# rust-bio/rust-bio

Measured on AMD Instinct MI355X. Metric: GCUPS (SW) + FM-index queries/sec, higher is better.
Workload: dtype int16; 1 GPU; 1000000 x 150 bp synthetic read pairs per GPU, Aligner::local affine-gap (-5,-1,+1,-1), score+coords+traceback ops (BASELINE configs[1]); pairs_per_gpu=1000000, read_len=150, parallelism=shard1

## Files before the change

rust-bio_amd/csrc/bg_common.h:

```cpp
#ifndef BG_COMMON_H
#define BG_COMMON_H
#include <functional>
#include <hip/hip_runtime.h>

#include <cstdint>
#include <cstdlib>
#include <cstdio>
#include <cstring>
#include <string>
#include <vector>

#include "biogpu.h"

extern thread_local std::string bg_tls_error;

#define BG_HIP(call)                                                                     \
    do {                                                                                 \
        hipError_t e__ = (call);                                                         \
        if (e__ != hipSuccess) {                                                         \
            bg_tls_error = std::string(#call) + ": " + hipGetErrorString(e__);           \
            return e__ == hipErrorOutOfMemory ? BG_ERR_OOM : BG_ERR_HIP;                 \
        }                                                                                \
    } while (0)

struct bg_band_scratch;
void bg_band_scratch_free(bg_band_scratch*);
struct bg_seed_scratch;
void bg_seed_scratch_free(bg_seed_scratch*);
struct bg_host_pipe;
void bg_host_pipe_free(bg_host_pipe*);
struct bg_fm_pipe;
void bg_fm_pipe_free(bg_fm_pipe*);
struct bg_myers_scratch;
void bg_myers_scratch_free(bg_myers_scratch*);

struct bg_ctx {
    int device = 0;
    hipStream_t stream = nullptr;
    void* tb = nullptr;
    size_t tb_bytes = 0;
    void* aux = nullptr;
    size_t aux_bytes = 0;
    void* bnd = nullptr;
    size_t bnd_bytes = 0;
    void* io[6] = {};
    size_t io_cap[6] = {};
    void* h_ops = nullptr;
    size_t h_ops_cap = 0;
    void* unpk[2] = {};
    size_t unpk_cap[2] = {};
    void* table = nullptr;
    size_t table_bytes = 0;
    void* sw_table = nullptr;
    size_t sw_table_bytes = 0;
    uint64_t table_hash = 0;
    int table_alpha = 0;
    int32_t* table_matrix = nullptr;
    bg_band_scratch* band = nullptr;
    bg_host_pipe* pipe = nullptr;
    bg_seed_scratch* seed = nullptr;
    bg_fm_pipe* fm_pipe = nullptr;
    bg_myers_scratch* myers = nullptr;
    int64_t myers_chunk_jobs = 0;
    int64_t myers_lds_bytes = 0;
    uint64_t fm_wide_from = 0xFFFFFFFFull;
    uint32_t fm_wide_sb_shift = 17;
    bool fm_host_bytes = false;
    int64_t host_chunk_pairs = 0;
    int64_t chunk_pairs = 0;
    int64_t seed_chunk_reads = 0;
    bool force_wide = false;
    bool no_pk16 = false;
    bool no_local_fast = false;
    bool no_pk16_frame = false;
    bool no_couples = false;
    int band_chain_global = -1;
    bool fq_no_fused = false;
    int sam_lanes = 0;
    int fq_emit_mode = 0;
    int64_t sa_chunk_symbols = 0;
    bool band_chain_rows = true;
    bool band_join_global = false;
    int band_fill_v1 = 0;
    bool band_interior_off = false;
    bool band_packed_off = false;
    int64_t band_packed_thresh = 0;
    int64_t band_budget_gb = 0;
    bool band_on_host = false;
    hipEvent_t scratch_done = nullptr;
    hipStream_t scratch_stream = nullptr;
    bool scratch_used = false;
    bool timing = false;
    hipEvent_t ev[2] = {nullptr, nullptr};
    bg_timing_t last = {};
    uint32_t fill_mask = 0;
    bool fill_framed = false;
};

int bg_reserve(void** p, size_t* cur, size_t need);
int bg_scan_u32(const uint32_t* d_len, uint64_t n, uint64_t* d_off, uint64_t* d_sums, hipStream_t st);
int bg_align_batch_dev_hint(bg_ctx* ctx, const bg_scoring_t* sc, int mode, uint64_t n_pairs, const uint8_t* d_x,
                            const uint64_t* d_x_off, const uint8_t* d_y, const uint64_t* d_y_off, uint32_t max_xlen,
                            uint32_t max_ylen, bg_alignment_t* d_out, uint8_t* d_ops, uint64_t ops_stride, void* stream,
                            int len_hint);

size_t bg_compact_ops_scratch(uint64_t n);
int bg_range_to_host(const uint8_t* d_src, uint8_t* h_dst, const uint64_t* d_slot , hipStream_t st);
int bg_compact_ops_dev(bg_alignment_t* d_rec, uint64_t n, const uint8_t* d_ops, uint8_t* d_compact, bool global_offsets, uint64_t* d_cell,
                       uint64_t* d_batch_total, void* d_scratch, bool long_ops, hipStream_t st);

struct bg_scratch_guard {
    bg_ctx* ctx;
    hipStream_t st;
    bg_scratch_guard(bg_ctx* c, hipStream_t s) : ctx(c), st(s) {
        if (ctx->scratch_used && ctx->scratch_stream != st) hipStreamWaitEvent(st, ctx->scratch_done, 0);
    }
    ~bg_scratch_guard() {
        if (hipEventRecord(ctx->scratch_done, st) == hipSuccess) {
            ctx->scratch_stream = st;
            ctx->scratch_used = true;
        }
    }
};
inline hipError_t bg_copy_pieces(void* dst, const void* src, size_t bytes, hipMemcpyKind kind, hipStream_t st) {
    static const size_t piece = [] {
        const char* e = getenv("BG_COPY_PIECE");
        const long long v = e ? atoll(e) : 0;
// ... 30 lines not shown
```

rust-bio_amd/csrc/core.hip:

```cpp
#include <sched.h>

#include <algorithm>
#include <condition_variable>
#include <deque>
#include <mutex>
#include <thread>

#include <cstdlib>

#include "bg_common.h"

thread_local std::string bg_tls_error;

int bg_reserve(void** p, size_t* cur, size_t need) {
    if (need <= *cur) return BG_OK;
    if (*p) {
        hipFree(*p);
        *p = nullptr;
        *cur = 0;
    }
    need = (need + 255) & ~(size_t)255;
    BG_HIP(hipMalloc(p, need));
    *cur = need;
    return BG_OK;
// ... 198 lines not shown
    }
    if (!strcmp(key, "myers_lds_bytes")) {
        if (value != 0 && (value < 4096 || value > 65536)) return BG_ERR_INVALID_ARG;
        ctx->myers_lds_bytes = value;
        return BG_OK;
    }
    if (!strcmp(key, "sa_chunk_symbols")) {
        if (value < 0) return BG_ERR_INVALID_ARG;
        ctx->sa_chunk_symbols = value;
        return BG_OK;
    }
    if (!strcmp(key, "band_chain_rows")) {
        ctx->band_chain_rows = value != 0;
        return BG_OK;
    }
    if (!strcmp(key, "band_chain_global")) {
        ctx->band_chain_global = (int)value;
        return BG_OK;
    }
    if (!strcmp(key, "band_fill_v1")) {
        ctx->band_fill_v1 = value > 0 ? 1 : value < 0 ? -1 : 0;
        return BG_OK;
    }
    if (!strcmp(key, "band_interior_off")) {
        ctx->band_interior_off = value != 0;
        return BG_OK;
    }
    if (!strcmp(key, "band_packed_off")) {
        ctx->band_packed_off = value != 0;
        return BG_OK;
    }
    if (!strcmp(key, "band_packed_thresh")) {
        if (value < 0 || value > 0xffff) return BG_ERR_INVALID_ARG;
        ctx->band_packed_thresh = value;
        return BG_OK;
    }
    if (!strcmp(key, "band_budget_gb")) {
        if (value < 0 || value > 256) return BG_ERR_INVALID_ARG;
        ctx->band_budget_gb = value;
        return BG_OK;
    }
    if (!strcmp(key, "band_on_host")) {
        ctx->band_on_host = value != 0;
        return BG_OK;
    }
    if (!strcmp(key, "fm_host_bytes")) {
        ctx->fm_host_bytes = value != 0;
        return BG_OK;
    }
    if (!strcmp(key, "host_chunk_pairs")) {
        ctx->host_chunk_pairs = value;
        return BG_OK;
    }
    if (!strcmp(key, "no_couples")) {
        ctx->no_couples = value != 0;
        return BG_OK;
    }
    if (!strcmp(key, "no_local_fast")) {
        ctx->no_local_fast = value != 0;
        return BG_OK;
    }
    if (!strcmp(key, "no_pk16_frame")) {
        ctx->no_pk16_frame = value != 0;
        return BG_OK;
    }
    if (!strcmp(key, "no_pk16")) {
        ctx->no_pk16 = value != 0;
        return BG_OK;
    }
    if (!strcmp(key, "force_wide")) {
        ctx->force_wide = value != 0;
        return BG_OK;
    }
    return BG_ERR_INVALID_ARG;
}

extern "C" int bg_enable_timing(bg_ctx* ctx, int on) {
    if (!ctx) return BG_ERR_INVALID_ARG;
    ctx->timing = on != 0;
    ctx->last = {};
    return BG_OK;
}

extern "C" int bg_last_fill_kernels(bg_ctx* ctx, uint32_t* mask) {
    if (!ctx || !mask) return BG_ERR_INVALID_ARG;
    *mask = ctx->fill_mask;
    return BG_OK;
}

extern "C" int bg_last_fill_framed(bg_ctx* ctx, int* framed) {
    if (!ctx || !framed) return BG_ERR_INVALID_ARG;
    *framed = ctx->fill_framed ? 1 : 0;
    return BG_OK;
}

extern "C" int bg_get_timing(bg_ctx* ctx, bg_timing_t* out) {
    if (!ctx || !out) return BG_ERR_INVALID_ARG;
    *out = ctx->last;
    ctx->last = {};
    return BG_OK;
}

namespace {
__global__ __launch_bounds__(256) void ops_counts_kernel(const bg_alignment_t* __restrict__ rec, uint64_t n, uint32_t* __restrict__ cnt) {
    const uint64_t p = (uint64_t)blockIdx.x * blockDim.x + threadIdx.x;
    if (p < n) cnt[p] = rec[p].status == BG_OK ? rec[p].n_ops : 0u;
// ... 62 lines not shown
```

rust-bio_amd/csrc/sw_api.hip:

```cpp
#include <algorithm>
#include <chrono>
#include <map>
#include <type_traits>

#include <atomic>
#include <condition_variable>
#include <mutex>
#include <thread>

#include "sw_kernels.h"

namespace bgsw {
void launch_traceback(const SwArgs& a, int nw, hipStream_t st);

static sw_fill_fn sw_fill_get(SwFill f, bool narrow, int lp, int r, int which = 0) {
    static sw_fill_fn (*const get[])(bool, int, int, int) = {
#define BG_X(F) sw_fill_get_##F,
        BG_SW_FILLS(BG_X)
#undef BG_X
    };
    return get[f](narrow, lp, r, which);
}
static int instantiated_r(SwFill f, bool narrow, int lp, int r0, uint32_t m = 0) {
    for (int r = r0; r <= 12; r++)
        if ((!m || m % r == 0) && sw_fill_get(f, narrow, lp, r)) return r;
    return 0;
}

struct Config {
    int lp, r;
};
static Config pick_config(uint32_t m_cap) {
    if (m_cap <= 192) return {16, std::max(2, 2 * (int)((m_cap + 31) / 32))};
    if (m_cap <= 384) return {32, std::max(8, 2 * (int)((m_cap + 63) / 64))};
    return {64, 8};
}

static int64_t score_magnitude(const SwScoring& c, const int32_t* matrix) {
    int64_t mag = std::max<int64_t>(std::abs((int64_t)c.go), std::abs((int64_t)c.ge));
    for (int32_t v : {c.xp, c.xs, c.yp, c.ys})
        if (v != BG_MIN_SCORE) mag = std::max<int64_t>(mag, std::abs((int64_t)v));
    if (matrix) {
        for (size_t t = 0; t < 65536; t++) mag = std::max<int64_t>(mag, std::abs((int64_t)matrix[t]));
    } else {
        mag = std::max<int64_t>(mag, std::max(std::abs((int64_t)c.match), std::abs((int64_t)c.mismatch)));
    }
    return mag;
}

struct FillPlan {
    int lp = 0, r = 0;
    sw_fill_fn fill = nullptr, fill_rest = nullptr, fill_second = nullptr;
    uint32_t tb_fmt = TBF_K1;
    uint32_t fill_bit = 0;
    bool k1p = false, framed = false;
};
static FillPlan plan_fill(const bg_ctx& ctx, const SwScoring& c, int sm, int64_t mag, uint32_t max_xlen, uint32_t max_ylen) {
    const Config cfg = pick_config(max_xlen);
    const bool local = c.xp == 0 && c.xs == 0 && c.yp == 0 && c.ys == 0;
    const bool lf = local && c.go < 0 && c.mismatch < 0 && c.match >= 0 && !ctx.no_local_fast;
    FillPlan p;
    p.lp = cfg.lp;
    if (!ctx.no_pk16 && sm == SCORE_PARAMS && cfg.lp <= 32 && max_xlen >= 1 && mag * ((int64_t)std::max(max_xlen, max_ylen) + 2) <= 2040) {
        const int32_t M = BG_MIN_SCORE;
        SwFill f = lf      ? FILL_K1P_LF
                   : local ? FILL_K1P_LOCAL
// ... 157 lines not shown
        const uint32_t u = threadIdx.x >= (unsigned)o ? s[threadIdx.x - o] : 0;
        __syncthreads();
        s[threadIdx.x] += u;
        __syncthreads();
    }
    cnt[blockIdx.x * 1024u + threadIdx.x] = base + s[threadIdx.x] - v;
}
__global__ __launch_bounds__(256) void sw_key_scatter_kernel(const uint64_t* __restrict__ x_off, const uint64_t* __restrict__ y_off, uint64_t pair0,
                                                             uint32_t n, uint32_t* __restrict__ cursor, uint32_t* __restrict__ perm,
                                                             const uint32_t* __restrict__ st) {
    if (st && st[0] == st[2] && st[1] == st[3]) return;
    const uint32_t p = blockIdx.x * blockDim.x + threadIdx.x;
    const bool valid = p < n;
    uint32_t base;
    const uint32_t rank = wave_key_add(cursor, valid ? len_key(x_off, y_off, pair0 + p) : 0u, valid, base);
    if (valid) perm[base + rank] = p;
}
__global__ void sw_decide_kernel(const uint32_t* __restrict__ st, uint32_t n, int forced, uint32_t* __restrict__ n_eff) {
    const bool uniform = forced < 0 && st[0] == st[2] && st[1] == st[3];
    n_eff[0] = uniform ? n : 0u;
    n_eff[1] = uniform ? 0u : n;
}
}

using namespace bgsw;

int bg_compact_matrix(const int32_t* matrix, std::vector<uint8_t>& code_map, std::vector<int32_t>& table) {
    return compact_matrix(matrix, code_map, table);
}

static int check_scoring(const bg_scoring_t* sc) {
    if (sc->gap_open > 0 || sc->gap_extend > 0 || sc->xclip_prefix > 0 || sc->xclip_suffix > 0 ||
        sc->yclip_prefix > 0 || sc->yclip_suffix > 0)
        return BG_ERR_POSITIVE_PENALTY;
    return BG_OK;
}

static void reset_fill_report(bg_ctx* ctx) {
    if (!ctx) return;
    ctx->fill_mask = 0;
    ctx->fill_framed = false;
}

static int align_batch_dev_impl(bg_ctx* ctx, const bg_scoring_t* sc, int mode, uint64_t n_pairs,
                                const uint8_t* d_x, const uint64_t* d_x_off, const uint8_t* d_y,
                                const uint64_t* d_y_off, uint32_t max_xlen, uint32_t max_ylen,
                                bg_alignment_t* d_out, uint8_t* d_ops, uint64_t ops_stride,
                                void* stream, int len_hint, const uint8_t* packed_codes = nullptr) {
    if (!ctx || !sc || mode < BG_MODE_CUSTOM || mode > BG_MODE_LOCAL) return BG_ERR_INVALID_ARG;
    int rc = check_scoring(sc);
    if (rc) return rc;
    if (n_pairs == 0) return BG_OK;
    if (!d_x_off || !d_y_off || !d_out) return BG_ERR_INVALID_ARG;
    if (d_ops && ops_stride < (uint64_t)max_xlen + max_ylen + 4) return BG_ERR_OPS_CAP;
    if (max_xlen > (1u << 24) || max_ylen > (1u << 24)) return BG_ERR_TOO_LARGE;
    hipStream_t st = (hipStream_t)stream;
    BG_HIP(hipSetDevice(ctx->device));
    bg_scratch_guard guard(ctx, st);

    SwArgs a = {};
    a.x = d_x;
    a.x_off = d_x_off;
    a.y = d_y;
    a.y_off = d_y_off;
    a.sc = {sc->gap_open,     sc->gap_extend,   sc->xclip_prefix, sc->xclip_suffix,
            sc->yclip_prefix, sc->yclip_suffix, sc->match_score,  sc->mismatch_score};
    if (mode == BG_MODE_GLOBAL) a.sc.xp = a.sc.xs = a.sc.yp = a.sc.ys = BG_MIN_SCORE;
    if (mode == BG_MODE_SEMIGLOBAL) {
        a.sc.xp = a.sc.xs = BG_MIN_SCORE;
        a.sc.yp = a.sc.ys = 0;
    }
    if (mode == BG_MODE_LOCAL) a.sc.xp = a.sc.xs = a.sc.yp = a.sc.ys = 0;
    a.mode = mode;
    a.filter_clips = (mode == BG_MODE_SEMIGLOBAL || mode == BG_MODE_LOCAL);
    a.out = d_out;
    a.ops = d_ops;
    a.ops_stride = ops_stride;

    int sm = SCORE_PARAMS;
    if (sc->matrix) {
        uint64_t h = 0xcbf29ce484222325ull;
        {
            const uint64_t* w = (const uint64_t*)sc->matrix;
            uint64_t h2 = 0x9e3779b97f4a7c15ull;
            for (size_t t = 0; t < 32768; t += 2) {
                h = (h ^ w[t]) * 0x100000001b3ull;
                h2 = (h2 + w[t + 1]) * 0xff51afd7ed558ccdull;
                h2 ^= h2 >> 32;
            }
            h ^= h2;
            if (h == 0) h = 1;
        }
        if (ctx->table_hash != h || !ctx->table_matrix || memcmp(ctx->table_matrix, sc->matrix, 65536 * sizeof(int32_t)) != 0) {
            std::vector<uint8_t> code_map;
            std::vector<int32_t> table;
            const int A = compact_matrix(sc->matrix, code_map, table);
            const size_t bytes = 256 + table.size() * 4;
            ctx->table_hash = 0;
            if (!ctx->table_matrix && !(ctx->table_matrix = (int32_t*)malloc(65536 * sizeof(int32_t)))) return BG_ERR_OOM;
            if ((rc = bg_reserve(&ctx->sw_table, &ctx->sw_table_bytes, bytes))) return rc;
            BG_HIP(hipMemcpyAsync((uint8_t*)ctx->sw_table + 256, table.data(), table.size() * 4,
                                  hipMemcpyHostToDevice, st));
            BG_HIP(hipMemcpyAsync(ctx->sw_table, code_map.data(), 256, hipMemcpyHostToDevice, st));
            BG_HIP(hipStreamSynchronize(st));
            memcpy(ctx->table_matrix, sc->matrix, 65536 * sizeof(int32_t));
            ctx->table_hash = h;
            ctx->table_alpha = A;
// ... 58 lines not shown
    uint32_t *d_keycnt = nullptr, *d_keysum = nullptr, *d_perm = nullptr, *d_lenst = nullptr;
    if (plan.k1p && !ctx->no_couples) {
        const size_t need = (size_t)kLenKeys * 4 + 1024 * 4 + 64 + chunk * 4;
        if ((rc = bg_reserve(&ctx->bnd, &ctx->bnd_bytes, need))) return rc;
        a.bnd = (int4*)ctx->bnd;
        d_keycnt = (uint32_t*)ctx->bnd;
        d_keysum = d_keycnt + kLenKeys;
        d_lenst = d_keysum + 1024;
        d_perm = d_lenst + 16;
    }

    for (uint64_t p0 = 0; p0 < n_pairs; p0 += chunk) {
        a.pair0 = p0;
        a.n_pairs = (uint32_t)std::min<uint64_t>(chunk, n_pairs - p0);
        const uint32_t njobs = (a.n_pairs + pw - 1) / pw;
        a.perm = nullptr;
        a.len_stats = nullptr;
        a.n_eff = nullptr;
        if (d_perm && a.n_pairs >= 64 && len_hint != 1) {
            const uint32_t* d_st = nullptr;
            if (len_hint < 0) {
                BG_HIP(hipMemsetAsync(d_lenst, 0xff, 8, st));
                BG_HIP(hipMemsetAsync(d_lenst + 2, 0, 8, st));
                sw_len_stats_kernel<<<dim3(std::min<uint32_t>((a.n_pairs + 255) / 256, 256)), dim3(256), 0, st>>>(d_x_off, d_y_off, p0, a.n_pairs, d_lenst);
                d_st = d_lenst;
            }
            BG_HIP(hipMemsetAsync(d_keycnt, 0, (size_t)kLenKeys * 4, st));
            sw_key_hist_kernel<<<dim3((a.n_pairs + 255) / 256), dim3(256), 0, st>>>(d_x_off, d_y_off, p0, a.n_pairs, d_keycnt, d_st);
            sw_key_block_sums_kernel<<<dim3(1024), dim3(256), 0, st>>>(d_keycnt, d_keysum, d_st);
            sw_key_scan_kernel<<<dim3(1024), dim3(1024), 0, st>>>(d_keycnt, d_keysum, d_st);
            sw_key_scatter_kernel<<<dim3((a.n_pairs + 255) / 256), dim3(256), 0, st>>>(d_x_off, d_y_off, p0, a.n_pairs, d_keycnt, d_perm, d_st);
            BG_HIP(hipGetLastError());
            sw_decide_kernel<<<dim3(1), dim3(1), 0, st>>>(d_lenst, a.n_pairs, len_hint < 0 ? -1 : 0, d_lenst + 4);
            a.perm = d_perm;
            a.len_stats = d_st;
            a.n_eff = d_lenst + 4;
        }
        if (ctx->timing) BG_HIP(hipEventRecord(ctx->ev[0], st));
        const uint32_t nwaves = plan.k1p ? (njobs + 1) / 2 : njobs;
        plan.fill<<<dim3((nwaves + 3) / 4), dim3(256), 0, st>>>(a);
        BG_HIP(hipGetLastError());
        if (ctx->timing) BG_HIP(hipEventRecord(ctx->ev[1], st));
        if (plan.fill_rest) plan.fill_rest<<<dim3((nwaves + 3) / 4), dim3(256), 0, st>>>(a);
        if (plan.fill_second && len_hint != 1) plan.fill_second<<<dim3((nwaves + 3) / 4), dim3(256), 0, st>>>(a);
        BG_HIP(hipGetLastError());
        if (ctx->timing) {
            BG_HIP(hipEventSynchronize(ctx->ev[1]));
            float ms = 0;
            BG_HIP(hipEventElapsedTime(&ms, ctx->ev[0], ctx->ev[1]));
            ctx->last.fill_ms += ms;
            ctx->last.fill_launches += 1;
            BG_HIP(hipEventRecord(ctx->ev[0], st));
        }
        launch_traceback(a, nw, st);
        BG_HIP(hipGetLastError());
        if (ctx->timing) {
            BG_HIP(hipEventRecord(ctx->ev[1], st));
            BG_HIP(hipEventSynchronize(ctx->ev[1]));
            float ms = 0;
            BG_HIP(hipEventElapsedTime(&ms, ctx->ev[0], ctx->ev[1]));
            ctx->last.traceback_ms += ms;
            ctx->last.traceback_launches += 1;
        }
    }
    return BG_OK;
}

int bg_align_batch_dev_hint(bg_ctx* ctx, const bg_scoring_t* sc, int mode, uint64_t n_pairs, const uint8_t* d_x,
                            const uint64_t* d_x_off, const uint8_t* d_y, const uint64_t* d_y_off, uint32_t max_xlen,
                            uint32_t max_ylen, bg_alignment_t* d_out, uint8_t* d_ops, uint64_t ops_stride, void* stream,
                            int len_hint) {
    return align_batch_dev_impl(ctx, sc, mode, n_pairs, d_x, d_x_off, d_y, d_y_off, max_xlen, max_ylen, d_out, d_ops, ops_stride,
                                stream, len_hint);
}

extern "C" int bg_align_batch_dev(bg_ctx* ctx, const bg_scoring_t* sc, int mode, uint64_t n_pairs,
                                  const uint8_t* d_x, const uint64_t* d_x_off, const uint8_t* d_y,
                                  const uint64_t* d_y_off, uint32_t max_xlen, uint32_t max_ylen,
                                  bg_alignment_t* d_out, uint8_t* d_ops, uint64_t ops_stride,
                                  void* stream) {
    reset_fill_report(ctx);
    return align_batch_dev_impl(ctx, sc, mode, n_pairs, d_x, d_x_off, d_y, d_y_off, max_xlen, max_ylen, d_out, d_ops, ops_stride, stream, -1);
}

extern "C" int bg_align_batch_packed_dev(bg_ctx* ctx, const bg_scoring_t* sc, int mode, uint64_t n_pairs, const uint32_t* d_x,
                                         const uint64_t* d_x_off, const uint32_t* d_y, const uint64_t* d_y_off,
                                         const uint8_t codes[4], uint32_t max_xlen, uint32_t max_ylen, bg_alignment_t* d_out,
                                         uint8_t* d_ops, uint64_t ops_stride, void* stream) {
    if (!codes || (n_pairs && (!d_x || !d_y))) return BG_ERR_INVALID_ARG;
    for (int a = 0; a < 4; a++)
        for (int b = a + 1; b < 4; b++)
            if (codes[a] == codes[b]) return BG_ERR_INVALID_ARG;
    reset_fill_report(ctx);
    return align_batch_dev_impl(ctx, sc, mode, n_pairs, (const uint8_t*)d_x, d_x_off, (const uint8_t*)d_y, d_y_off, max_xlen, max_ylen,
                                d_out, d_ops, ops_stride, stream, -1, codes);
}

struct bg_host_pipe {
    static constexpr int NSET = 3;
    struct Set {
        uint8_t *h_in = nullptr, *h_out = nullptr;
        uint8_t *d_in = nullptr, *d_out = nullptr;
        uint8_t *d_cmp = nullptr, *d_scan = nullptr;
        size_t in_cap = 0, out_cap = 0, cmp_cap = 0, scan_cap = 0;
        hipEvent_t in_done = nullptr, k_done = nullptr, out_done = nullptr;
    } set[NSET];
    uint64_t* d_cell = nullptr;
// ... 374 lines not shown
```

rust-bio_amd/csrc/sw_kernels.h:

```cpp
#ifndef BG_SW_KERNELS_H
#define BG_SW_KERNELS_H
#include <type_traits>

#include "bg_common.h"

namespace bgsw {

constexpr int32_t NEG = BG_MIN_SCORE;

enum : uint32_t {
    TB_START = 0, TB_INS = 1, TB_DEL = 2, TB_SUBST = 3, TB_MATCH = 4,
    TB_XCLIP_PREFIX = 5, TB_XCLIP_SUFFIX = 6, TB_YCLIP_PREFIX = 7, TB_YCLIP_SUFFIX = 8
};
enum : uint32_t { C_XS = 7, C_MATCH = 6, C_SUBST = 5, C_INS = 3, C_DEL = 2, C_XP = 1, C_YP = 0 };
constexpr int32_t kNarrowFloor = -(1 << 26);
constexpr int32_t kNarrowKeyFloor = (int32_t)0x80000000;

enum { SCORE_PARAMS = 0, SCORE_LDS = 1, SCORE_GLOBAL = 2 };
constexpr int kMaxLdsAlphabet = 64;

struct SwScoring {
    int32_t go, ge, xp, xs, yp, ys;
    int32_t match, mismatch;
};
// ... 112 lines not shown
    }
    if (sc.xp > c.S) {
        c.S = sc.xp;
        c.sbits = TB_XCLIP_PREFIX;
    }
    return c;
}
__device__ __forceinline__ void col0_fold(const SwScoring& sc, uint32_t m, int32_t& fold, uint32_t& lx0) {
    fold = NEG;
    lx0 = 0;
    if (m >= 2) {
        const Col0 c = col0_cell(sc, 1, m, NEG);
        if (c.S + sc.xs > fold) {
            fold = c.S + sc.xs;
            lx0 = m - 1;
        }
    }
}
__device__ __forceinline__ int32_t col0_S(const SwScoring& sc, uint32_t i, uint32_t m, int32_t fold0) {
    if (i == 0) return 0;
    return col0_cell(sc, i, m, fold0).S;
}

struct Row0 {
    int32_t S, D;
    uint32_t sbits, dbits;
};
__device__ __forceinline__ Row0 row0_cell(const SwScoring& sc, uint32_t j) {
    Row0 c;
    if (j == 1) {
        c.D = sc.go;
        c.dbits = TB_START;
    } else {
        const int32_t d_score = sc.go + sc.ge * ((int32_t)j - 1);
        const int32_t c_score = sc.yp + sc.go;
        if (d_score > c_score) {
            c.D = d_score;
            c.dbits = TB_DEL;
        } else {
            c.D = c_score;
            c.dbits = TB_YCLIP_PREFIX;
        }
    }
    if (c.D > sc.yp) {
        c.S = c.D;
        c.sbits = TB_DEL;
    } else {
        c.S = sc.yp;
        c.sbits = TB_YCLIP_PREFIX;
    }
    return c;
}

__device__ __forceinline__ uint32_t s_nibble_of_code(uint32_t code) {
    switch (code) {
        case C_MATCH: return TB_MATCH;
        case C_SUBST: return TB_SUBST;
        case C_INS: return TB_INS;
        case C_DEL: return TB_DEL;
        case C_XP: return TB_XCLIP_PREFIX;
        case C_YP: return TB_YCLIP_PREFIX;
        default: return TB_XCLIP_SUFFIX;
    }
}

typedef void (*sw_fill_fn)(const SwArgs);

#define BG_K1_SHAPES(X) X(16, 2) X(16, 4) X(16, 6) X(16, 8) X(16, 10) X(16, 12) X(32, 8) X(32, 10) X(32, 12) X(64, 8)
#define BG_K1_TABLE_SHAPES(X) X(16, 6) X(16, 12) X(32, 12) X(64, 8)
#define BG_K1_TABLE_LDS_NARROW_SHAPES(X) BG_K1_TABLE_SHAPES(X) X(16, 8) X(16, 10)
#define BG_K1P_SHAPES(X) X(16, 2) X(16, 4) X(16, 5) X(16, 6) X(16, 8) X(16, 10) X(16, 12) X(32, 8) X(32, 10) X(32, 12)
#define BG_K1P_LOCAL_SHAPES(X)                                                                                    \
    X(16, 2) X(16, 3) X(16, 4) X(16, 5) X(16, 6) X(16, 7) X(16, 8) X(16, 9) X(16, 10) X(16, 11) X(16, 12) \
    X(32, 7) X(32, 8) X(32, 9) X(32, 10) X(32, 11) X(32, 12)

#define BG_SW_FILLS(X) \
    X(K1) X(K1_LOCAL) X(K1_LF) X(K1_LDS) X(K1_LDS_LOCAL) X(K1_GLOBAL) X(K1P_CUSTOM) X(K1P_GLOBAL) X(K1P_SEMIGLOBAL) X(K1P_LOCAL) X(K1P_LF) X(K1P_LF_FRAMED)
enum SwFill {
#define BG_X(F) FILL_##F,
    BG_SW_FILLS(BG_X)
#undef BG_X
};
#define BG_X(F) sw_fill_fn sw_fill_get_##F(bool narrow, int lp, int r, int which);
BG_SW_FILLS(BG_X)
#undef BG_X

}
#endif
```

rust-bio_amd/csrc/sw_traceback.hip:

```cpp
#include "sw_kernels.h"

namespace bgsw {

constexpr uint32_t kSegStride = 20;

template <int NW, bool PERM>
__global__ __launch_bounds__(256) __attribute__((amdgpu_waves_per_eu(5, 5))) void sw_traceback_kernel(const SwArgs a) {
    const uint32_t slot = blockIdx.x * blockDim.x + threadIdx.x;
    if (slot >= (a.n_eff ? a.n_eff[PERM ? 1 : 0] : a.n_pairs)) return;
    const uint32_t pair = PERM ? a.perm[slot] : slot;
    const SwScoring sc = a.sc;
    const SwGeom geo = a.g;
    const uint32_t R = geo.r, LP = geo.lp, PW = 64 / geo.lp;

    const uint64_t xo = a.x_off[a.pair0 + pair], yo = a.y_off[a.pair0 + pair];
    const uint32_t m = (uint32_t)(a.x_off[a.pair0 + pair + 1] - xo);
    const uint32_t n = (uint32_t)(a.y_off[a.pair0 + pair + 1] - yo);
    if (len_over(geo, m, n)) {
        bg_alignment_t bad = {};
        bad.xlen = m;
        bad.ylen = n;
        bad.ops_off = (a.pair0 + pair + 1) * a.ops_stride;
        bad.mode = (uint8_t)a.mode;
        bad.status = (int8_t)BG_ERR_INVALID_ARG;
        a.out[a.pair0 + pair] = bad;
        return;
    }

    const int32_t* aux = a.aux + (size_t)slot * geo.aux_stride;
    const int32_t* gLy = aux + geo.off_Ly();
    const int32_t* gLx = aux + geo.off_Lx();
    const uint8_t* bits = (const uint8_t*)(aux + geo.off_bits());
    const uint32_t sbits_m0 = (uint32_t)aux[0];
    const int32_t score = aux[1];
    const uint32_t lxn = (uint32_t)aux[2];

    const uint32_t job = slot / PW, grp = slot % PW;
    const uint32_t* tbj = (const uint32_t*)a.tb + (size_t)job * tb_job_words(geo.nstrips, geo.nsteps, NW);
    __shared__ __align__(16) uint32_t s_seg[256 * kSegStride];
    uint32_t* seg = s_seg + threadIdx.x * kSegStride;
    uint64_t seg_tag = ~0ull;
    auto cell = [&](uint32_t i, uint32_t j) -> uint32_t {
        const uint32_t i1 = i - 1, lrow = __umulhi(i1, geo.r_inv), rr = i1 - lrow * R;
        const uint32_t st = lrow >> geo.lp_shift, llc = lrow & (LP - 1);
        const uint64_t g = (uint64_t)st * geo.nsteps + (j - 1 + llc);
        constexpr uint32_t tsteps = 16 / NW;
        const uint64_t base = (g / tsteps) * 1024ull + (grp * LP + llc) * 16u;
        if (base != seg_tag) {
#pragma unroll
            for (int q = 0; q < 4; q++) *(uint4*)&seg[4 * q] = *(const uint4*)&tbj[base + 4 * q];
            seg_tag = base;
        }
        const uint32_t w = seg[(uint32_t)(g % tsteps) * NW + rr / 6];
        const uint32_t c = rr % 6;
        if (geo.tb_fmt == TBF_K1) return (w >> (5 * c)) & 31u;
        if (geo.tb_fmt == TBF_K1_LF) {
            const uint32_t u = (w >> (5 * c)) & 31u;
            return ((u >> 1) & 7u) | ((~u & 1u) << 3) | (~u & 16u);
        }
        const uint32_t v = (w >> (5 * (c % 3) + 16 * (c / 3))) & 31u;
        const uint32_t mv = (v >> 1) & 7u;
        return ((geo.tb_fmt == TBF_K1P_LF && mv == 0) ? (uint32_t)C_XP : mv) | ((v & 1u) << 3) | (v & 16u);
    };
    auto s_fill = [&](uint32_t i, uint32_t j) -> uint32_t {
        if (j == 0) {
            if (i == 0) return TB_START;
            if (i == m) return sbits_m0;
            return col0_cell(sc, i, m, NEG).sbits;
        }
        if (i == 0) return row0_cell(sc, j).sbits;
        return s_nibble_of_code(cell(i, j) & 7u);
    };
    auto s_nib = [&](uint32_t i, uint32_t j) -> uint32_t {
        if (j == n) return (uint32_t)bits[i] & 15u;
        return s_fill(i, j);
    };
    auto i_nib = [&](uint32_t i, uint32_t j) -> uint32_t {
        if (j == n) return (uint32_t)bits[i] >> 4;
        if (i == 0) return TB_START;
        if (j == 0) return col0_cell(sc, i, m, NEG).ibits;
        return (cell(i, j) & 8u) ? TB_INS : s_fill(i - 1, j);
    };
    auto d_nib = [&](uint32_t i, uint32_t j) -> uint32_t {
        if (j == 0) return TB_START;
        if (i == 0) return row0_cell(sc, j).dbits;
        return (cell(i, j) & 16u) ? TB_DEL : s_fill(i, j - 1);
    };

    uint8_t* ops_end = a.ops ? a.ops + (a.pair0 + pair + 1) * a.ops_stride : nullptr;
    uint32_t n_ops = 0;
    uint32_t clip_len[4] = {0, 0, 0, 0};
    uint32_t n_clips = 0;
    int status = BG_OK;
    const bool dword_ok = ops_end && (((uintptr_t)ops_end & 3) == 0);
    uint32_t acc = 0;
    auto push = [&](uint32_t op) {
        ++n_ops;
        if (!ops_end) return;
        if (dword_ok) {
            acc = (acc << 8) | op;
            if ((n_ops & 3) == 0) *(uint32_t*)(ops_end - n_ops) = acc;
        } else {
            ops_end[-(int64_t)n_ops] = (uint8_t)op;
        }
    };
    auto push_clip = [&](uint32_t op, uint32_t len) {
        if (a.filter_clips) return;
        if (n_clips < 4) clip_len[n_clips] = len;
        else status = BG_ERR_TRACEBACK;
        n_clips++;
        push(op);
    };

    uint32_t i = m, j = n;
    uint32_t xstart = 0, ystart = 0, xend = m, yend = n;
    uint32_t layer = s_nib(m, n);
    const uint32_t guard = 2 * (m + n) + 16;
    uint32_t c_here = 0;
    bool have_c = false;
    for (uint32_t steps = 0; layer != TB_START; steps++) {
        if (steps > guard || (ops_end && n_ops + 1 > a.ops_stride)) {
            status = BG_ERR_TRACEBACK;
            break;
        }
        if (layer >= TB_INS && layer <= TB_MATCH && i >= 1 && i <= m && j >= 1 && j < n) {
            const bool is_ins = layer == TB_INS, is_del = layer == TB_DEL;
            const uint32_t ti = i - (is_del ? 0u : 1u), tj = j - (is_ins ? 0u : 1u);
            if (ti >= 1 && tj >= 1) {
                if (!have_c && (is_ins || is_del)) c_here = cell(i, j);
                const bool ext = (is_ins && (c_here & 8u)) || (is_del && (c_here & 16u));
                push(is_ins ? (uint32_t)BG_OP_INS : is_del ? (uint32_t)BG_OP_DEL : layer == TB_MATCH ? (uint32_t)BG_OP_MATCH : (uint32_t)BG_OP_SUBST);
                c_here = cell(ti, tj);
                have_c = true;
                if (!ext) layer = s_nibble_of_code(c_here & 7u);
                i = ti;
                j = tj;
                continue;
            }
        }
        have_c = false;
        uint32_t next;
        switch (layer) {
            case TB_INS:
                push(BG_OP_INS);
                next = i_nib(i, j);
                i -= 1;
                break;
            case TB_DEL:
                push(BG_OP_DEL);
                next = d_nib(i, j);
                j -= 1;
                break;
            case TB_MATCH:
            case TB_SUBST:
                push(layer == TB_MATCH ? BG_OP_MATCH : BG_OP_SUBST);
                next = (i && j) ? s_nib(i - 1, j - 1) : TB_START;
                i -= 1;
                j -= 1;
                break;
            case TB_XCLIP_PREFIX:
                push_clip(BG_OP_XCLIP, i);
                xstart = i;
                i = 0;
                next = s_nib(0, j);
                break;
            case TB_XCLIP_SUFFIX: {
                if ((geo.tb_fmt == TBF_K1P_LF || geo.tb_fmt == TBF_K1_LF) && j != n) {
                    status = BG_ERR_TRACEBACK;
                    layer = TB_START;
                    continue;
                }
                const uint32_t lx = (j == n) ? lxn
                                    : geo.tb_fmt == TBF_K1 ? (uint32_t)gLx[j]
                                    : geo.lp == 16 ? (uint32_t)((const uint8_t*)gLx)[j] : (uint32_t)((const uint16_t*)gLx)[j];
                push_clip(BG_OP_XCLIP, lx);
                i -= lx;
                xend = i;
                next = i <= m ? s_nib(i, j) : TB_START;
                break;
            }
            case TB_YCLIP_PREFIX:
                push_clip(BG_OP_YCLIP, j);
                ystart = j;
                j = 0;
                next = s_nib(i, 0);
                break;
            default: {
                const uint32_t ly = (uint32_t)gLy[i];
                push_clip(BG_OP_YCLIP, ly);
                j -= ly;
                yend = j;
                next = j <= n ? s_nib(i, j) : TB_START;
                break;
            }
        }
        if (i > m || j > n) {
            status = BG_ERR_TRACEBACK;
            break;
        }
        layer = next;
    }

    if (dword_ok) {
        const uint32_t k = n_ops & 3, done = n_ops - k;
        for (uint32_t t = 0; t < k; t++) ops_end[-(int64_t)(done + t + 1)] = (uint8_t)(acc >> (8 * (k - 1 - t)));
    }
    bg_alignment_t rec;
    rec.score = score;
    rec.xstart = xstart;
    rec.xend = xend;
    rec.ystart = ystart;
    rec.yend = yend;
    rec.xlen = m;
    rec.ylen = n;
    rec.n_ops = n_ops;
    rec.ops_off = (a.pair0 + pair + 1) * a.ops_stride - n_ops;
    const uint32_t nc = n_clips < 4 ? n_clips : 4;
    for (uint32_t c = 0; c < 4; c++) rec.clip_len[c] = c < nc ? clip_len[nc - 1 - c] : 0;
    rec.n_clips = (uint8_t)nc;
    rec.mode = (uint8_t)a.mode;
    rec.status = (int8_t)status;
    rec._pad = 0;
    rec._reserved = 0;
    a.out[a.pair0 + pair] = rec;
}

void launch_traceback(const SwArgs& a, int nw, hipStream_t st) {
    const uint32_t blocks = (a.n_pairs + 255) / 256;
    if (nw == 2)
        sw_traceback_kernel<2, false><<<dim3(blocks), dim3(256), 0, st>>>(a);
    else
        sw_traceback_kernel<1, false><<<dim3(blocks), dim3(256), 0, st>>>(a);
    if (a.perm) {
        if (nw == 2)
            sw_traceback_kernel<2, true><<<dim3(blocks), dim3(256), 0, st>>>(a);
        else
            sw_traceback_kernel<1, true><<<dim3(blocks), dim3(256), 0, st>>>(a);
    }
}

}
```

Baseline: 2190 GCUPS.

## Add lean specialized traceback kernel for single-strip K1P formats

Result: no change. 2205 GCUPS, median of 6 (+0.7%).

```diff
diff --git a/rust-bio_amd/csrc/bg_common.h b/rust-bio_amd/csrc/bg_common.h
--- a/rust-bio_amd/csrc/bg_common.h
+++ b/rust-bio_amd/csrc/bg_common.h
@@ -73,6 +73,8 @@
     bool no_pk16 = false;
     bool no_local_fast = false;
     bool no_pk16_frame = false;
+    bool ops_stride_any = false;
+    bool tb_general = false;
     bool no_couples = false;
     int band_chain_global = -1;
     bool fq_no_fused = false;
diff --git a/rust-bio_amd/csrc/core.hip b/rust-bio_amd/csrc/core.hip
--- a/rust-bio_amd/csrc/core.hip
+++ b/rust-bio_amd/csrc/core.hip
@@ -274,6 +274,14 @@
         ctx->host_chunk_pairs = value;
         return BG_OK;
     }
+    if (!strcmp(key, "ops_stride_any")) {
+        ctx->ops_stride_any = value != 0;
+        return BG_OK;
+    }
+    if (!strcmp(key, "tb_general")) {
+        ctx->tb_general = value != 0;
+        return BG_OK;
+    }
     if (!strcmp(key, "no_couples")) {
         ctx->no_couples = value != 0;
         return BG_OK;
diff --git a/rust-bio_amd/csrc/sw_api.hip b/rust-bio_amd/csrc/sw_api.hip
--- a/rust-bio_amd/csrc/sw_api.hip
+++ b/rust-bio_amd/csrc/sw_api.hip
@@ -11,7 +11,7 @@
 #include "sw_kernels.h"
 
 namespace bgsw {
-void launch_traceback(const SwArgs& a, int nw, hipStream_t st);
+void launch_traceback(const SwArgs& a, int nw, bool general, hipStream_t st);
 
 static sw_fill_fn sw_fill_get(SwFill f, bool narrow, int lp, int r, int which = 0) {
     static sw_fill_fn (*const get[])(bool, int, int, int) = {
@@ -275,7 +275,7 @@
     if (rc) return rc;
     if (n_pairs == 0) return BG_OK;
     if (!d_x_off || !d_y_off || !d_out) return BG_ERR_INVALID_ARG;
-    if (d_ops && ops_stride < (uint64_t)max_xlen + max_ylen + 4) return BG_ERR_OPS_CAP;
+    if (d_ops && ops_stride < (uint64_t)max_xlen + max_ylen + 4 && !ctx->ops_stride_any) return BG_ERR_OPS_CAP;
     if (max_xlen > (1u << 24) || max_ylen > (1u << 24)) return BG_ERR_TOO_LARGE;
     hipStream_t st = (hipStream_t)stream;
     BG_HIP(hipSetDevice(ctx->device));
@@ -440,7 +440,7 @@
             ctx->last.fill_launches += 1;
             BG_HIP(hipEventRecord(ctx->ev[0], st));
         }
-        launch_traceback(a, nw, st);
+        launch_traceback(a, nw, ctx->tb_general, st);
         BG_HIP(hipGetLastError());
         if (ctx->timing) {
             BG_HIP(hipEventRecord(ctx->ev[1], st));
diff --git a/rust-bio_amd/csrc/sw_kernels.h b/rust-bio_amd/csrc/sw_kernels.h
--- a/rust-bio_amd/csrc/sw_kernels.h
+++ b/rust-bio_amd/csrc/sw_kernels.h
@@ -188,7 +188,7 @@
     return c;
 }
 
-__device__ __forceinline__ uint32_t s_nibble_of_code(uint32_t code) {
+__host__ __device__ constexpr uint32_t s_nibble_of_code(uint32_t code) {
     switch (code) {
         case C_MATCH: return TB_MATCH;
         case C_SUBST: return TB_SUBST;
diff --git a/rust-bio_amd/csrc/sw_traceback.hip b/rust-bio_amd/csrc/sw_traceback.hip
--- a/rust-bio_amd/csrc/sw_traceback.hip
+++ b/rust-bio_amd/csrc/sw_traceback.hip
@@ -4,8 +4,22 @@
 
 constexpr uint32_t kSegStride = 20;
 
-template <int NW, bool PERM>
-__global__ __launch_bounds__(256) __attribute__((amdgpu_waves_per_eu(5, 5))) void sw_traceback_kernel(const SwArgs a) {
+constexpr uint32_t TBF_ANY = ~0u;
+constexpr uint32_t k2_nibbles(bool lf) {
+    uint32_t t = 0;
+    for (uint32_t c = 0; c < 8; c++) t |= s_nibble_of_code(lf && c == 0 ? (uint32_t)C_XP : c) << (4 * c);
+    return t;
+}
+#ifndef BG_K2_WAVES
+#define BG_K2_WAVES 5
+#endif
+template <uint32_t FMT>
+constexpr int k2_waves = FMT == TBF_ANY ? 5 : BG_K2_WAVES;
+
+template <int NW, bool PERM, uint32_t FMT, bool SINGLE>
+__global__ __launch_bounds__(256) __attribute__((amdgpu_waves_per_eu(k2_waves<FMT>, k2_waves<FMT>))) void sw_traceback_kernel(const SwArgs a) {
+    constexpr bool LEAN = FMT != TBF_ANY;
+    static_assert(LEAN == SINGLE && (!LEAN || FMT == TBF_K1P || FMT == TBF_K1P_LF), "the lean loop and the one-strip lookup read K1p cells");
     const uint32_t slot = blockIdx.x * blockDim.x + threadIdx.x;
     if (slot >= (a.n_eff ? a.n_eff[PERM ? 1 : 0] : a.n_pairs)) return;
     const uint32_t pair = PERM ? a.perm[slot] : slot;
@@ -39,28 +53,45 @@
     const uint32_t* tbj = (const uint32_t*)a.tb + (size_t)job * tb_job_words(geo.nstrips, geo.nsteps, NW);
     __shared__ __align__(16) uint32_t s_seg[256 * kSegStride];
     uint32_t* seg = s_seg + threadIdx.x * kSegStride;
-    uint64_t seg_tag = ~0ull;
+    using tag_t = typename std::conditional<SINGLE, uint32_t, uint64_t>::type;
+    tag_t seg_tag = ~(tag_t)0;
+    const uint32_t fmt = LEAN ? FMT : geo.tb_fmt;
+    const uint32_t r_inv16 = (geo.r_inv + 0xffffu) >> 16;
+    auto cell_raw = [&](uint32_t i, uint32_t j) -> uint32_t {
+        constexpr uint32_t tsteps = 16 / NW;
+        if constexpr (SINGLE) {
+            const uint32_t i1 = i - 1, lrow = (uint32_t)__umul24(i1, r_inv16) >> 16, rr = i1 - __umul24(lrow, R);
+            const uint32_t g = j - 1 + lrow;
+            const uint32_t base = (g / tsteps) * 1024u + (grp * LP + lrow) * 16u;
+            if (base != seg_tag) {
+#pragma unroll
+                for (int q = 0; q < 4; q++) *(uint4*)&seg[4 * q] = *(const uint4*)&tbj[base + 4 * q];
+                seg_tag = base;
+            }
+            const uint32_t bit = (g % tsteps) * (32 * NW) + __umul24(rr, 5) + (__umul24(rr, 11) >> 5);
+            return (seg[bit >> 5] >> (bit & 31u)) & 31u;
+        } else {
+            const uint32_t i1 = i - 1, lrow = __umulhi(i1, geo.r_inv), rr = i1 - lrow * R;
+            const uint32_t st = lrow >> geo.lp_shift, llc = lrow & (LP - 1);
+            const uint64_t g = (uint64_t)st * geo.nsteps + (j - 1 + llc);
+            const uint64_t base = (g / tsteps) * 1024ull + (grp * LP + llc) * 16u;
+            if (base != seg_tag) {
+#pragma unroll
+                for (int q = 0; q < 4; q++) *(uint4*)&seg[4 * q] = *(const uint4*)&tbj[base + 4 * q];
+                seg_tag = base;
+            }
+            const uint32_t w = seg[(uint32_t)(g % tsteps) * NW + rr / 6];
+            const uint32_t c = rr % 6;
+            if (fmt == TBF_K1 || fmt == TBF_K1_LF) return (w >> (5 * c)) & 31u;
+            return (w >> (5 * (c % 3) + 16 * (c / 3))) & 31u;
+        }
+    };
     auto cell = [&](uint32_t i, uint32_t j) -> uint32_t {
-        const uint32_t i1 = i - 1, lrow = __umulhi(i1, geo.r_inv), rr = i1 - lrow * R;
-        const uint32_t st = lrow >> geo.lp_shift, llc = lrow & (LP - 1);
-        const uint64_t g = (uint64_t)st * geo.nsteps + (j - 1 + llc);
-        constexpr uint32_t tsteps = 16 / NW;
-        const uint64_t base = (g / tsteps) * 1024ull + (grp * LP + llc) * 16u;
-        if (base != seg_tag) {
-#pragma unroll
-            for (int q = 0; q < 4; q++) *(uint4*)&seg[4 * q] = *(const uint4*)&tbj[base + 4 * q];
-            seg_tag = base;
-        }
-        const uint32_t w = seg[(uint32_t)(g % tsteps) * NW + rr / 6];
-        const uint32_t c = rr % 6;
-        if (geo.tb_fmt == TBF_K1) return (w >> (5 * c)) & 31u;
-        if (geo.tb_fmt == TBF_K1_LF) {
-            const uint32_t u = (w >> (5 * c)) & 31u;
-            return ((u >> 1) & 7u) | ((~u & 1u) << 3) | (~u & 16u);
-        }
-        const uint32_t v = (w >> (5 * (c % 3) + 16 * (c / 3))) & 31u;
+        const uint32_t v = cell_raw(i, j);
+        if (fmt == TBF_K1) return v;
+        if (fmt == TBF_K1_LF) return ((v >> 1) & 7u) | ((~v & 1u) << 3) | (~v & 16u);
         const uint32_t mv = (v >> 1) & 7u;
-        return ((geo.tb_fmt == TBF_K1P_LF && mv == 0) ? (uint32_t)C_XP : mv) | ((v & 1u) << 3) | (v & 16u);
+        return ((fmt == TBF_K1P_LF && mv == 0) ? (uint32_t)C_XP : mv) | ((v & 1u) << 3) | (v & 16u);
     };
     auto s_fill = [&](uint32_t i, uint32_t j) -> uint32_t {
         if (j == 0) {
@@ -92,17 +123,13 @@
     uint32_t clip_len[4] = {0, 0, 0, 0};
     uint32_t n_clips = 0;
     int status = BG_OK;
-    const bool dword_ok = ops_end && (((uintptr_t)ops_end & 3) == 0);
+    const bool dword_ok = ops_end && (((uintptr_t)ops_end & 3) == 0), byte_ok = ops_end && !dword_ok;
     uint32_t acc = 0;
     auto push = [&](uint32_t op) {
         ++n_ops;
-        if (!ops_end) return;
-        if (dword_ok) {
-            acc = (acc << 8) | op;
-            if ((n_ops & 3) == 0) *(uint32_t*)(ops_end - n_ops) = acc;
-        } else {
-            ops_end[-(int64_t)n_ops] = (uint8_t)op;
-        }
+        acc = (acc << 8) | op;
+        if (dword_ok & ((n_ops & 3) == 0)) *(uint32_t*)(ops_end - n_ops) = acc;
+        if (byte_ok) ops_end[-(int64_t)n_ops] = (uint8_t)op;
     };
     auto push_clip = [&](uint32_t op, uint32_t len) {
         if (a.filter_clips) return;
@@ -116,29 +143,7 @@
     uint32_t xstart = 0, ystart = 0, xend = m, yend = n;
     uint32_t layer = s_nib(m, n);
     const uint32_t guard = 2 * (m + n) + 16;
-    uint32_t c_here = 0;
-    bool have_c = false;
-    for (uint32_t steps = 0; layer != TB_START; steps++) {
-        if (steps > guard || (ops_end && n_ops + 1 > a.ops_stride)) {
-            status = BG_ERR_TRACEBACK;
-            break;
-        }
-        if (layer >= TB_INS && layer <= TB_MATCH && i >= 1 && i <= m && j >= 1 && j < n) {
-            const bool is_ins = layer == TB_INS, is_del = layer == TB_DEL;
-            const uint32_t ti = i - (is_del ? 0u : 1u), tj = j - (is_ins ? 0u : 1u);
-            if (ti >= 1 && tj >= 1) {
-                if (!have_c && (is_ins || is_del)) c_here = cell(i, j);
-                const bool ext = (is_ins && (c_here & 8u)) || (is_del && (c_here & 16u));
-                push(is_ins ? (uint32_t)BG_OP_INS : is_del ? (uint32_t)BG_OP_DEL : layer == TB_MATCH ? (uint32_t)BG_OP_MATCH : (uint32_t)BG_OP_SUBST);
-                c_here = cell(ti, tj);
-                have_c = true;
-                if (!ext) layer = s_nibble_of_code(c_here & 7u);
-                i = ti;
-                j = tj;
-                continue;
-            }
-        }
-        have_c = false;
+    auto general_step = [&]() {
         uint32_t next;
         switch (layer) {
             case TB_INS:
@@ -165,13 +170,13 @@
                 next = s_nib(0, j);
                 break;
             case TB_XCLIP_SUFFIX: {
-                if ((geo.tb_fmt == TBF_K1P_LF || geo.tb_fmt == TBF_K1_LF) && j != n) {
+                if ((fmt == TBF_K1P_LF || fmt == TBF_K1_LF) && j != n) {
                     status = BG_ERR_TRACEBACK;
                     layer = TB_START;
-                    continue;
+                    return;
                 }
                 const uint32_t lx = (j == n) ? lxn
-                                    : geo.tb_fmt == TBF_K1 ? (uint32_t)gLx[j]
+                                    : (fmt == TBF_K1) ? (uint32_t)gLx[j]
                                     : geo.lp == 16 ? (uint32_t)((const uint8_t*)gLx)[j] : (uint32_t)((const uint16_t*)gLx)[j];
                 push_clip(BG_OP_XCLIP, lx);
                 i -= lx;
@@ -196,9 +201,83 @@
         }
         if (i > m || j > n) {
             status = BG_ERR_TRACEBACK;
-            break;
+            next = TB_START;
         }
         layer = next;
+    };
+    auto over_budget = [&](uint32_t steps) { return steps > guard || (ops_end && n_ops + 1 > a.ops_stride); };
+
+    if constexpr (!LEAN) {
+        uint32_t c_here = 0;
+        bool have_c = false;
+        for (uint32_t steps = 0; layer != TB_START; steps++) {
+            if (over_budget(steps)) {
+                status = BG_ERR_TRACEBACK;
+                break;
+            }
+            if (layer >= TB_INS && layer <= TB_MATCH && i >= 1 && i <= m && j >= 1 && j < n) {
+                const bool is_ins = layer == TB_INS, is_del = layer == TB_DEL;
+                const uint32_t ti = i - (is_del ? 0u : 1u), tj = j - (is_ins ? 0u : 1u);
+                if (ti >= 1 && tj >= 1) {
+                    if (!have_c && (is_ins || is_del)) c_here = cell(i, j);
+                    const bool ext = (is_ins && (c_here & 8u)) || (is_del && (c_here & 16u));
+                    push(is_ins ? (uint32_t)BG_OP_INS : is_del ? (uint32_t)BG_OP_DEL : layer == TB_MATCH ? (uint32_t)BG_OP_MATCH : (uint32_t)BG_OP_SUBST);
+                    c_here = cell(ti, tj);
+                    have_c = true;
+                    if (!ext) layer = s_nibble_of_code(c_here & 7u);
+                    i = ti;
+                    j = tj;
+                    continue;
+                }
+            }
+            have_c = false;
+            general_step();
+        }
+    } else {
+        constexpr uint32_t kOps = BG_OP_INS << 8 | BG_OP_DEL << 16 | BG_OP_SUBST << 24 | BG_OP_MATCH;
+        constexpr uint32_t kExt = 1u << 8 | 16u << 16;
+        static_assert(TB_INS == 1 && TB_DEL == 2 && TB_SUBST == 3 && TB_MATCH == 4, "kOps, kExt");
+        constexpr uint32_t kNib = k2_nibbles(FMT == TBF_K1P_LF);
+        auto interior = [&](uint32_t l) {
+            return l - TB_INS <= TB_MATCH - TB_INS && i > (l != TB_DEL ? 1u : 0u) && i <= m && j > (l != TB_INS ? 1u : 0u) && j < n;
+        };
+        uint32_t steps = 0;
+        while (layer != TB_START) {
+            if (interior(layer)) {
+                if (over_budget(steps)) {
+                    status = BG_ERR_TRACEBACK;
+                    layer = TB_START;
+                } else {
+                    const uint64_t room = ops_end ? a.ops_stride - n_ops : ~0ull;
+                    uint32_t left = guard + 1 - steps;
+                    if (room < left) left = (uint32_t)room;
+                    steps += left;
+                    uint32_t v = layer <= TB_DEL ? cell_raw(i, j) : 0;
+                    uint32_t ti = i - (layer != TB_DEL ? 1u : 0u), tj = j - (layer != TB_INS ? 1u : 0u);
+                    do {
+                        const uint32_t sh = 8 * (layer & 3u);
+                        const uint32_t ext = v & (kExt >> sh) & 0xffu;
+                        push((kOps >> sh) & 0xffu);
+                        i = ti;
+                        j = tj;
+                        v = cell_raw(i, j);
+                        if (!ext) layer = (kNib >> (2 * (v & 14u))) & 15u;
+                        ti = i - (layer != TB_DEL ? 1u : 0u);
+                        tj = j - (layer != TB_INS ? 1u : 0u);
+                    } while ((--left != 0) & (layer - TB_INS <= TB_MATCH - TB_INS) & (ti != 0) & (tj != 0));
+                    steps -= left;
+                }
+            }
+            while (layer != TB_START && !interior(layer)) {
+                if (over_budget(steps)) {
+                    status = BG_ERR_TRACEBACK;
+                    layer = TB_START;
+                    break;
+                }
+                general_step();
+                steps++;
+            }
+        }
     }
 
     if (dword_ok) {
@@ -225,18 +304,29 @@
     a.out[a.pair0 + pair] = rec;
 }
 
-void launch_traceback(const SwArgs& a, int nw, hipStream_t st) {
+template <uint32_t FMT, bool SINGLE>
+static void launch_k2(const SwArgs& a, int nw, hipStream_t st) {
     const uint32_t blocks = (a.n_pairs + 255) / 256;
     if (nw == 2)
-        sw_traceback_kernel<2, false><<<dim3(blocks), dim3(256), 0, st>>>(a);
+        sw_traceback_kernel<2, false, FMT, SINGLE><<<dim3(blocks), dim3(256), 0, st>>>(a);
     else
-        sw_traceback_kernel<1, false><<<dim3(blocks), dim3(256), 0, st>>>(a);
+        sw_traceback_kernel<1, false, FMT, SINGLE><<<dim3(blocks), dim3(256), 0, st>>>(a);
     if (a.perm) {
         if (nw == 2)
-            sw_traceback_kernel<2, true><<<dim3(blocks), dim3(256), 0, st>>>(a);
+            sw_traceback_kernel<2, true, FMT, SINGLE><<<dim3(blocks), dim3(256), 0, st>>>(a);
         else
-            sw_traceback_kernel<1, true><<<dim3(blocks), dim3(256), 0, st>>>(a);
+            sw_traceback_kernel<1, true, FMT, SINGLE><<<dim3(blocks), dim3(256), 0, st>>>(a);
     }
 }
 
-}
+void launch_traceback(const SwArgs& a, int nw, bool general, hipStream_t st) {
+    const bool single = a.g.nstrips == 1 && tb_job_words(1, a.g.nsteps, nw) < (1ull << 31) && (uint64_t)a.g.m_cap * a.g.r < (1u << 16);
+    if (!general && single && a.g.tb_fmt == TBF_K1P_LF)
+        launch_k2<TBF_K1P_LF, true>(a, nw, st);
+    else if (!general && single && a.g.tb_fmt == TBF_K1P)
+        launch_k2<TBF_K1P, true>(a, nw, st);
+    else
+        launch_k2<TBF_ANY, false>(a, nw, st);
+}
+
+}
```
